# wjmaddox/online_gp

Hardware: AMD Instinct MI355X
Metric: streaming updates/sec (WISKI, 50^3 inducing grid) (higher is better)
Workload: dtype f32

## Files before the change

online_gp_amd/csrc/solve.hip:

```cpp
#include "pcg.h"

#include <hip/hip_ext.h>

#include <chrono>
#include <cstdlib>
#include <map>
#include <mutex>
#include <vector>

static struct WiskiProf {
  bool on = false;
  bool armed = false;
  std::vector<hipEvent_t> ev;
  size_t used = 0;
  unsigned long long* d_stamp = nullptr;
  size_t stamp_pairs = 0, stamp_used = 0;
  struct Span { size_t off, n; };
  std::vector<Span> spans;
} g_prof;
constexpr unsigned long long PROF_CLOCK_MASK = 0xffffffffffffull;
constexpr size_t PROF_STAMP_ARENA_PAIRS = (size_t)1 << 20;

extern "C" int wiski_prof_start(int max_launches) {
  if (max_launches < 1) return WISKI_E_BADARG;
// ... 1831 lines not shown
  return WISKI_OK;
}

template <typename real>
static int pcg_iterate(const PcgPlan<real>& plan) {
  const GridDev<real>& G = plan.G;
  const PcgArgs<real>& a = plan.a;
  const PcgLayout<real>& L = plan.L;
  const PcgScal& S = L.S;
  const hipStream_t s = plan.s;
  const int m = plan.m, k = plan.k, max_iter = a.max_iter;
  const double tol2 = plan.tol2;
  const bool spectral = plan.path.spectral;
  real *const r = plan.r, *const p = L.p, *const pt = L.pt, *const hp = L.hp, *const cpart = plan.cpart;
  const int cnch = plan.cnch, czl = plan.czl;
  wiski_pcg_async* const as = a.handle;
  int mode = a.mode, first_check = a.first_check;
  const int check_every = a.check_every < 1 ? 10 : a.check_every;
  int rc = WISKI_OK;

  std::vector<double> h_rn0(k), h_rn(k);
  double err_seen = 0;
  int dev = 0;
  if (hipGetDevice(&dev) != hipSuccess) return WISKI_E_LAUNCH;
  std::unique_lock<std::mutex> poll_lock(g_poll_mu, std::defer_lock);
  WiskiPoll* Pp = nullptr;
  if (as) {
    if (!as->poll) as->poll = new WiskiPoll();
    Pp = static_cast<WiskiPoll*>(as->poll);
  } else {
    poll_lock.lock();
    Pp = &g_polls[dev];
  }
  WiskiPoll& P = *Pp;
  if (poll_reserve(P, k) != WISKI_OK) return WISKI_E_LAUNCH;
  auto collect = [&]() {
    for (int c = 0; c < k; ++c) {
      h_rn0[c] = P.h[1 + c];
      h_rn[c] = P.h[1 + k + c];
    }
    err_seen = P.h[1 + 2 * k];
  };
  bool deferred = false;
  auto fetch = [&](int slot, long long queued_seq = 0) -> int {
    long long seq = queued_seq;
    if (!seq) {
      seq = ++P.seq;
      hipLaunchKernelGGL(k_pcg_publish, dim3(1), dim3(64), 0, s, S, slot, P.d, a.d_err, seq, tol2, P.g);
    }
    if (hipGetLastError() != hipSuccess) return WISKI_E_LAUNCH;
    if (mode == 1) {
      as->state = 1;
      as->it = slot;
      as->seq = seq;
      deferred = true;
      return WISKI_OK;
    }
    if (int prc = poll_wait(P, seq, s)) return prc;
    collect();
    return WISKI_OK;
  };
  auto converged = [&]() {
    for (int c = 0; c < k; ++c)
      if (h_rn0[c] > 0 && h_rn[c] > tol2 * h_rn0[c]) return false;
    return true;
  };

  int it = 0;
  bool done = false;
  if (mode == 2) {
    it = as->it;
    as->state = 0;
    if (int prc = poll_wait(P, as->seq, s)) return prc;
    collect();
    as->guard_ok = (long long)P.h[2 + 2 * k] == as->seq ? 1 : 0;
    done = converged();
    first_check = it;
    mode = 0;
  }
  if (first_check < 1) first_check = check_every;
  if (first_check > max_iter) first_check = max_iter;
  auto due = [&](int i) { return i == max_iter || i == first_check || (i > first_check && (i - first_check) % check_every == 0); };
  bool pending = false;
  auto flush_update = [&](bool publish = false) -> long long {
    long long seq = 0;
    if (pending) {
      if (publish) seq = ++P.seq;
      hipLaunchKernelGGL((k_pcg_update_x<real, 4>), plan.vgrid, dim3(256), 0, s, m, it - 1, tol2, (const real*)p, (const real*)pt, (const real*)hp,
                         cpart, cnch, czl, a.U, a.Z, r, S, publish ? P.d : (double*)nullptr, a.d_err, seq, P.g);
      pending = false;
    }
    return seq;
  };
  while (!done && it < max_iter) {
    if (plan.path.fused_cg) {
      constexpr bool fuse_upd = sizeof(real) == 4;
      if (!fuse_upd) flush_update();
      const bool init_now = plan.init_in_fwd && it == 0;
      rc = launch_spectral_fused_cg<real>(G, a.evec, a.evec2, a.eval, a.kscale, a.shift, r, k, L.sa, L.sb, it, pending ? 1 : 0, tol2, p, pt, cpart, cnch,
                                          czl, a.U, a.Z, S, s, init_now ? a.RHS : (const real*)nullptr, a.two_level);
      pending = false;
      if (rc) return rc;
      rc = plan.product_wide(p, pt, (real)1, S.php(it));
      if (rc) return rc;
      pending = true;
      ++it;
      if (due(it)) {
        rc = fetch(it, flush_update(true));
        if (rc) return rc;
        if (deferred) return WISKI_PENDING;
        done = converged();
      }
      continue;
    }
    if (spectral) {
      rc = launch_spectral_precond<real>(G, a.evec, a.evec2, a.eval, a.kscale, a.shift, r, k, L.sa, L.sb, L.ty, S.rho(it), s);
      if (rc) return rc;
      PCG_VEC_LAUNCH(plan, k_pcg_update_p, m, it, tol2, (const real*)(L.ty + (int64_t)k * m), (const real*)L.ty, p, pt, S);
    } else {
      rc = launch_kron<real>(G, a.tcol, r, k, a.kscale, L.tmp, L.y, r, S.rho(it), s);
      if (rc) return rc;
      PCG_VEC_LAUNCH(plan, k_pcg_update_p, m, it, tol2, (const real*)L.y, (const real*)r, p, pt, S);
    }
    rc = plan.product(p, pt, (real)1, S.php(it));
    if (rc) return rc;
    const bool pub = due(it + 1);
    const long long useq = pub ? ++P.seq : 0;
    PCG_VEC_LAUNCH(plan, k_pcg_update_x, m, it, tol2, (const real*)p, (const real*)pt, (const real*)hp, cpart, cnch, czl, a.U, a.Z, r, S,
                   pub ? P.d : (double*)nullptr, a.d_err, useq, P.g);
    ++it;
    if (due(it)) {
      rc = fetch(it, useq);
      if (rc) return rc;
      if (deferred) return WISKI_PENDING;
      done = converged();
    }
  }
  flush_update();
  if (hipGetLastError() != hipSuccess) return WISKI_E_LAUNCH;
  if (it == 0) {
    rc = fetch(0);
    if (rc) return rc;
  }
  if (a.h_iters) *a.h_iters = it;
  if (a.h_err) *a.h_err = (int32_t)err_seen;
  if (a.h_relres)
    for (int c = 0; c < k; ++c) a.h_relres[c] = h_rn0[c] > 0 ? sqrt(h_rn[c] / h_rn0[c]) : 0.0;
  return done ? WISKI_OK : WISKI_E_NOTCONV;
}
#undef PCG_VEC_LAUNCH

template <typename real>
int pcg(const wiski_grid* grid, const PcgArgs<real>& a, void* stream) {
  GridDev<real> G;
  int rc = make_grid_dev<real>(grid, &G);
  if (rc) return rc;
  const PcgPath path(G, a);
  rc = pcg_validate(G, a, path);
  if (rc) return rc;
  const PcgPlan<real> plan(G, a, path, (hipStream_t)stream);
  if (a.mode != 2) rc = pcg_start(plan);
  return rc ? rc : pcg_iterate(plan);
}
template int pcg<float>(const wiski_grid*, const PcgArgs<float>&, void*);
template int pcg<double>(const wiski_grid*, const PcgArgs<double>&, void*);

template <typename real>
static int spmv_impl(const wiski_grid* grid, const real* d_A, const real* d_V, int32_t k, const real* d_add, real beta, real* d_out, void* stream) {
  GridDev<real> G;
  int rc = make_grid_dev<real>(grid, &G);
  if (rc) return rc;
  if (!d_A || !d_V || !d_out || k < 1) return WISKI_E_BADARG;
  hipStream_t s = (hipStream_t)stream;
  if (G.m % 4 != 0) return launch_spmv<real>(G, d_A, d_V, k, d_add, beta, d_out, nullptr, s);
  const int nch = spmv_nch(G.d);
  const int64_t km = (int64_t)k * G.m;
  real* part = nullptr;
  if (hipMallocAsync((void**)&part, (size_t)nch * km * sizeof(real), s) != hipSuccess) return WISKI_E_LAUNCH;
  rc = launch_spmv4<real>(G, d_A, d_V, k, part, nullptr, (real)0, nullptr, s);
  if (rc == WISKI_OK) {
    int64_t blocks = (km + 255) / 256;
    if (blocks > 4096) blocks = 4096;
    hipLaunchKernelGGL((k_spmv_reduce<real>), dim3((unsigned)blocks), dim3(256), 0, s, km, nch, part, d_add, beta, d_out, 0);
    if (hipGetLastError() != hipSuccess) rc = WISKI_E_LAUNCH;
  }
  (void)hipFreeAsync(part, s);
  return rc;
}

template <typename real>
static int spmv_sym_impl(const wiski_grid* grid, const real* d_A, const real* d_V, int32_t k, const real* d_add, real beta, real* d_out, void* stream) {
// ... 147 lines not shown
```

online_gp_amd/csrc/spectral.hip:

```cpp
#include "wiski_common.h"

#include <atomic>

#ifdef SPEC_TIMING
__device__ long long g_spec_dbg[16];
#define SPEC_STAMP(i) do { if (threadIdx.x == 0 && blockIdx.x == 0 && blockIdx.y == 0) g_spec_dbg[i] = clock64(); } while (0)
#else
#define SPEC_STAMP(i) do {} while (0)
#endif
#ifndef SPEC_ABLATE
#ifndef SPEC_ST
#define SPEC_ST 32
#endif
#define SPEC_ABLATE 0
#endif

template <typename real>
struct V4 { real v[4]; };

template <typename real>
__device__ __forceinline__ V4<real> lds_read4(const real* p) {
  V4<real> r;
  if constexpr (sizeof(real) == 4) {
    float4 t = *reinterpret_cast<const float4*>(p);
// ... 810 lines not shown
          const unsigned long long mx = sMask[x];
          if ((mx >> y) & 1ull) {
            eidx[a][cc][r] = sPre[x] + __popcll(mx & ((1ull << y) - 1ull));
            f1v[a][cc][r] = 1.f / lam;
            f2v[a][cc][r] = 1.f;
            any_sel = true;
          }
        }
      }
    }
  for (; c < k; c += gridDim.y) {
    const int cn = c + gridDim.y;
    const bool more = cn < k;
    if (more) tX.issue(src + (int64_t)cn * m + (int64_t)i0 * g1 * g2, g1, g2);
    float dv[2][2][4];
    if constexpr (TL) {
      if (any_sel) {
#pragma unroll
        for (int a = 0; a < RT; ++a)
#pragma unroll
          for (int cc = 0; cc < 2; ++cc)
#pragma unroll
            for (int r = 0; r < 4; ++r) dv[a][cc][r] = eidx[a][cc][r] >= 0 ? dS[(int64_t)c * tl.r + eidx[a][cc][r]] : 0.f;
      }
    }
    spec_mfma_product<false, false, KS, RT>(sV1, bufA, wr, wc, lane, acc);
    store_tiles(bufB, SPEC_LDN);
    __syncthreads();
    spec_mfma_product<true, false, KS, RT>(bufB, sV2, wr, wc, lane, acc);
    spec_f32x4 c3[2][2];
    float rho_lane = 0.f;
#pragma unroll
    for (int a = 0; a < RT; ++a)
#pragma unroll
      for (int cc = 0; cc < 2; ++cc)
#pragma unroll
        for (int r = 0; r < 4; ++r) {
          float v = acc[a][cc][r];
          bool sel = false;
          if constexpr (TL) sel = any_sel && eidx[a][cc][r] >= 0;
          if (sel) v = dv[a][cc][r];
          else rho_lane += f2v[a][cc][r] * v * v;
          c3[a][cc][r] = v;
          acc[a][cc][r] = v * f1v[a][cc][r];
        }
    store_tiles(bufA, SPEC_LDN);
    if (rho != nullptr) {
      const double tot = block_reduce_sum((double)rho_lane, s_red);
      if (t == 0) unsafeAtomicAdd(rho + c, tot);
    }
    __syncthreads();
#pragma unroll
    for (int h = 0; h < 2; ++h) {
      spec_mfma_product<true, true, KS, RT>(bufA, sB2[h], wr, wc, lane, acc);
      store_tiles(bufB, SPEC_LDT);
      __syncthreads();
      if (h == 0) {
#pragma unroll
        for (int a = 0; a < RT; ++a)
#pragma unroll
          for (int cc = 0; cc < 2; ++cc)
#pragma unroll
            for (int r = 0; r < 4; ++r) acc[a][cc][r] = c3[a][cc][r] * f2v[a][cc][r];
        store_tiles(bufA, SPEC_LDN);
      } else if (more) {
        tX.commit(bufA, SPEC_LDT);
      }
      spec_mfma_product<true, false, KS, RT>(sB1[h], bufB, wr, wc, lane, acc);
      float* __restrict__ os = dst + ((int64_t)h * k + c) * m + (int64_t)i0 * g1 * g2;
#pragma unroll
      for (int a = 0; a < RT; ++a)
#pragma unroll
        for (int cc = 0; cc < 2; ++cc)
#pragma unroll
          for (int r = 0; r < 4; ++r) {
            const int x = wr * 16 * RT + a * 16 + l4 * 4 + r, y = wc * 32 + cc * 16 + l15;
            if (x < g1 && y < g2) os[x * g2 + y] = acc[a][cc][r];
          }
      __syncthreads();
    }
  }
}

template <int KS, int VW, int MODE>
__global__ __launch_bounds__(256) void k_spec_mode0_mfma(GridDev<float> G, const float* __restrict__ Va, const float* __restrict__ Vb, int split,
                                                         int transposed, const float* __restrict__ src, float* __restrict__ dst,
                                                         const float* __restrict__ rvec, int dot_c0, double* __restrict__ dots, int k, int it,
                                                         float* __restrict__ p, float* __restrict__ pt, PcgScal S, int apply, double tol2,
                                                         float* __restrict__ part, int nch, int zl, float* __restrict__ u, float* __restrict__ z) {
  __shared__ __attribute__((aligned(16))) float sF[64 * SPEC_LDT];
  __shared__ __attribute__((aligned(16))) float sIn[64 * SPEC_LDT];
  __shared__ double s_red[16];
  const int g0 = G.g[0], Sf = G.stride[0], m = G.m;
  const int cc = blockIdx.y;
  const int ntile = (Sf + 31) >> 5, per = (ntile + 7) >> 3;
  const int tile = (int)(blockIdx.x & 7) * per + (int)(blockIdx.x >> 3);
  if (tile >= ntile) return;
  const int s0 = tile * 32;
  const int t = threadIdx.x, lane = t & 63, w = t >> 6, wr = w >> 1, wc = w & 1;
  const int l15 = lane & 15, l4 = lane >> 4;
  const float* __restrict__ V0;
  int c = cc;
  float bt = 0.f;
  if (MODE == 1) {
    const int half = cc / k;
    c = cc - half * k;
    V0 = half == 0 ? Va : Vb;
    if (it > 0) {
      const double den = S.rho(it - 1)[c];
      bt = (float)(den > 0 ? S.rho(it)[c] / den : 0.0);
    }
  } else {
    V0 = cc < split ? Va : Vb;
  }
  SpecTile<VW> tV;
  tV.issue(V0, g0, g0);
  float4 tin[2];
  float al = 0.f;
  if (MODE == 2 && apply == 1) {
    const double den = S.php_sum(it - 1, cc);
    if (blockIdx.x == 0) pcg_dot_clear(S.php(it), cc, 1, S.k);
    if (pcg_active(S, it - 1, cc, tol2) && den > 0) al = (float)(S.rho(it - 1)[cc] / den);
  }
  float rn_part = 0.f, rhs_part = 0.f;
#pragma unroll
  for (int q = 0; q < 2; ++q) {
    const int b = (t >> 3) + 32 * q, q4 = (t & 7) * 4;
    const bool ok = b < g0 && s0 + q4 < Sf;
    const int64_t e = (int64_t)cc * m + (ok ? (int64_t)b * Sf + s0 + q4 : 0);
    tin[q] = *reinterpret_cast<const float4*>(src + e);
    if (!ok) tin[q] = make_float4(0.f, 0.f, 0.f, 0.f);
    if (MODE == 2 && apply == 2 && ok) {
      const float4 f4 = *reinterpret_cast<const float4*>(p + e), rv = tin[q];
      rhs_part += f4.x * f4.x + f4.y * f4.y + f4.z * f4.z + f4.w * f4.w;
      rn_part += rv.x * rv.x + rv.y * rv.y + rv.z * rv.z + rv.w * rv.w;
    }
    if (MODE == 2 && apply == 1 && ok) {
      const int64_t km = (int64_t)S.k * m;
      const float4 pv = *reinterpret_cast<const float4*>(p + e), ptv = *reinterpret_cast<const float4*>(pt + e);
      float4 uv = *reinterpret_cast<const float4*>(u + e), zv = *reinterpret_cast<const float4*>(z + e);
      float4 pp[8];
#pragma unroll
      for (int ch = 0; ch < 8; ++ch)
        if (ch < nch) pp[ch] = *reinterpret_cast<const float4*>(part + (int64_t)ch * km + e);
      if (zl) *reinterpret_cast<float4*>(part + (int64_t)(nch - 1) * km + e) = make_float4(0.f, 0.f, 0.f, 0.f);
      float4 hv = ptv;
#pragma unroll
      for (int ch = 0; ch < 8; ++ch)
        if (ch < nch) { hv.x += pp[ch].x; hv.y += pp[ch].y; hv.z += pp[ch].z; hv.w += pp[ch].w; }
      uv.x += al * pv.x; uv.y += al * pv.y; uv.z += al * pv.z; uv.w += al * pv.w;
      zv.x += al * ptv.x; zv.y += al * ptv.y; zv.z += al * ptv.z; zv.w += al * ptv.w;
      float4 rv = tin[q];
      rv.x -= al * hv.x; rv.y -= al * hv.y; rv.z -= al * hv.z; rv.w -= al * hv.w;
      rn_part += rv.x * rv.x + rv.y * rv.y + rv.z * rv.z + rv.w * rv.w;
      *reinterpret_cast<float4*>(u + e) = uv;
      *reinterpret_cast<float4*>(z + e) = zv;
      *reinterpret_cast<float4*>(const_cast<float*>(src) + e) = rv;
      tin[q] = rv;
    }
  }
  if (MODE == 2 && apply) {
    const double tot = block_reduce_sum((double)rn_part, s_red);
    if (t == 0) unsafeAtomicAdd(S.rn(it) + cc, tot);
    if (apply == 2) {
      const double tot0 = block_reduce_sum((double)rhs_part, s_red);
      if (t == 0) unsafeAtomicAdd(S.rn0() + cc, tot0);
    }
  }
  tV.commit(sF, transposed ? SPEC_LDN : SPEC_LDT);
#pragma unroll
  for (int q = 0; q < 2; ++q) *reinterpret_cast<float4*>(sIn + ((t >> 3) + 32 * q) * SPEC_LDT + (t & 7) * 4) = tin[q];
  __syncthreads();
  spec_f32x4 acc[2];
#pragma unroll
  for (int a = 0; a < 2; ++a)
#pragma unroll
    for (int r = 0; r < 4; ++r) acc[a][r] = 0.f;
  {
    const float* qb = sIn + l4 * SPEC_LDT + wc * 16 + l15;
    float af[KS][2], bf[KS];
    if (transposed) {
      const float* qa = sF + (wr * 32 + l15) * SPEC_LDN + l4;
#pragma unroll
      for (int i = 0; i < KS; ++i) { af[i][0] = qa[4 * i]; af[i][1] = qa[4 * i + 16 * SPEC_LDN]; }
    } else {
      const float* qa = sF + l4 * SPEC_LDT + wr * 32 + l15;
#pragma unroll
      for (int i = 0; i < KS; ++i) { af[i][0] = qa[4 * i * SPEC_LDT]; af[i][1] = qa[4 * i * SPEC_LDT + 16]; }
    }
#pragma unroll
    for (int i = 0; i < KS; ++i) bf[i] = qb[4 * i * SPEC_LDT];
#pragma unroll
    for (int i = 0; i < KS; ++i) {
      acc[0] = __builtin_amdgcn_mfma_f32_16x16x4f32(af[i][0], bf[i], acc[0], 0, 0, 0);
      acc[1] = __builtin_amdgcn_mfma_f32_16x16x4f32(af[i][1], bf[i], acc[1], 0, 0, 0);
    }
  }
  const int sidx = s0 + wc * 16 + l15;
  const bool dot = MODE == 0 && dots != nullptr && cc >= dot_c0;
  float dpart = 0.f;
  if (sidx < Sf) {
    float* __restrict__ tgt = MODE == 1 ? (cc < k ? pt : p) + (int64_t)c * m : dst + (int64_t)cc * m;
#pragma unroll
    for (int a = 0; a < 2; ++a)
#pragma unroll
      for (int r = 0; r < 4; ++r) {
        const int x = wr * 32 + a * 16 + l4 * 4 + r;
        if (x < g0) {
          const int64_t e = (int64_t)x * Sf + sidx;
          float o = acc[a][r];
          if (MODE == 1 && it > 0) o += bt * tgt[e];
          tgt[e] = o;
          if (dot) dpart += rvec[(int64_t)(cc - dot_c0) * m + e] * o;
        }
      }
  }
  if (dot) {
    const double tot = block_reduce_sum((double)dpart, s_red);
    if (t == 0) unsafeAtomicAdd(dots + (cc - dot_c0), tot);
  }
}

#define SPEC_DISPATCH_KS_VW(gmax, even, CALL) \
  do {                                        \
    if (even) {                               \
      if ((gmax) <= 16) CALL(4, 2);           \
      else if ((gmax) <= 32) CALL(8, 2);      \
      else if ((gmax) <= 48) CALL(12, 2);     \
      else if ((gmax) <= 52) CALL(13, 2);     \
      else CALL(16, 2);                       \
    } else {                                  \
      if ((gmax) <= 16) CALL(4, 1);           \
      else if ((gmax) <= 32) CALL(8, 1);      \
      else if ((gmax) <= 48) CALL(12, 1);     \
      else if ((gmax) <= 52) CALL(13, 1);     \
      else CALL(16, 1);                       \
    }                                         \
  } while (0)

template <typename real>
__global__ void k_spec_mode0_bwd_updp(GridDev<real> G, const real* __restrict__ X0, const real* __restrict__ Z0, const real* __restrict__ src, int k,
                                      int it, real* __restrict__ p, real* __restrict__ pt, PcgScal S);

template <typename real, bool DOT>
static int launch_mode0(const GridDev<real>& G, const real* Va, const real* Vb, int split, int transposed, const real* src, real* dst, int ncols,
                        const real* rvec, int dot_c0, double* dots, hipStream_t s) {
  const int g0 = G.g[0], Sf = G.stride[0];
  if constexpr (sizeof(real) == 4) {
    dim3 grd((unsigned)(8 * (((Sf + 31) / 32 + 7) / 8)), (unsigned)ncols);
#define M0(KS, VW)                                                                                                                          \
  hipLaunchKernelGGL((k_spec_mode0_mfma<KS, VW, 0>), grd, dim3(256), 0, s, G, Va, Vb, split, transposed, src, dst, rvec, dot_c0,            \
                     DOT ? dots : (double*)nullptr, 0, 0, (float*)nullptr, (float*)nullptr, PcgScal{nullptr, 0, nullptr}, 0, 0.0,         \
                     (float*)nullptr, 0, 0, (float*)nullptr, (float*)nullptr)
    SPEC_DISPATCH_KS_VW(g0, g0 % 2 == 0, M0);
#undef M0
  } else {
    const int P0 = (g0 + 3) & ~3;
    const size_t sh0 = (size_t)(P0 * P0 + P0 * SPEC_ST) * sizeof(real);
    hipLaunchKernelGGL((k_spec_mode0<real, DOT>), dim3((unsigned)((Sf + SPEC_ST - 1) / SPEC_ST), (unsigned)ncols), dim3(128), sh0, s, G, Va, Vb, split,
                       transposed, src, dst, rvec, dot_c0, dots);
  }
  return hipGetLastError() == hipSuccess ? WISKI_OK : WISKI_E_LAUNCH;
}

static int launch_mode0_fwd_upd(const GridDev<float>& G, const float* V0, float* r, float* dst, int k, int it, int apply, double tol2, float* p,
                                float* pt, float* part, int nch, int zl, float* u, float* z, PcgScal S, hipStream_t s) {
  const int g0 = G.g[0], Sf = G.stride[0];
  dim3 grd((unsigned)(8 * (((Sf + 31) / 32 + 7) / 8)), (unsigned)k);
#define M2(KS, VW)                                                                                                                        \
  hipLaunchKernelGGL((k_spec_mode0_mfma<KS, VW, 2>), grd, dim3(256), 0, s, G, V0, V0, 0, 0, (const float*)r, dst, (const float*)nullptr, 0, \
                     (double*)nullptr, k, it, p, pt, S, apply, tol2, part, nch, zl, u, z)
  SPEC_DISPATCH_KS_VW(g0, g0 % 2 == 0, M2);
#undef M2
  return hipGetLastError() == hipSuccess ? WISKI_OK : WISKI_E_LAUNCH;
}

template <typename real>
static int launch_mode0_bwd_updp(const GridDev<real>& G, const real* X0, const real* Z0, const real* src, int k, int it, real* p, real* pt,
                                 PcgScal S, hipStream_t s) {
  const int g0 = G.g[0], Sf = G.stride[0];
  if constexpr (sizeof(real) == 4) {
    dim3 grd((unsigned)(8 * (((Sf + 31) / 32 + 7) / 8)), (unsigned)(2 * k));
#define M1(KS, VW)                                                                                                                       \
  hipLaunchKernelGGL((k_spec_mode0_mfma<KS, VW, 1>), grd, dim3(256), 0, s, G, Z0, X0, 0, 1, src, (float*)nullptr, (const float*)nullptr, 0, \
                     (double*)nullptr, k, it, p, pt, S, 0, 0.0, (float*)nullptr, 0, 0, (float*)nullptr, (float*)nullptr)
    SPEC_DISPATCH_KS_VW(g0, g0 % 2 == 0, M1);
#undef M1
  } else {
    const int P0 = (g0 + 3) & ~3;
    const size_t sh0 = (size_t)(P0 * P0 + P0 * SPEC_ST) * sizeof(real);
    hipLaunchKernelGGL((k_spec_mode0_bwd_updp<real>), dim3((unsigned)((Sf + SPEC_ST - 1) / SPEC_ST), (unsigned)(2 * k)), dim3(128), sh0, s, G, X0, Z0,
                       src, k, it, p, pt, S);
  }
  return hipGetLastError() == hipSuccess ? WISKI_OK : WISKI_E_LAUNCH;
}

static int spec_cu_count() {
  static int n = 0;
  if (n == 0) {
    int dev = 0, v = 0;
    if (hipGetDevice(&dev) == hipSuccess && hipDeviceGetAttribute(&v, hipDeviceAttributeMultiprocessorCount, dev) == hipSuccess && v > 0) n = v;
    else n = 256;
  }
  return n;
}

constexpr size_t SPEC_SLAB_MFMA_LDS = (size_t)(4 * 64 * SPEC_LDT + 2 * 64 * SPEC_LDN) * sizeof(float);

template <typename real>
static int launch_slab(const GridDev<real>& G, const real* V1, const real* V2, const real* Z1, const real* Z2, const real* evals, real kscale,
                       real shift, const real* src, real* dst, int k, double* rho, hipStream_t s, const wiski_twolevel* two_level = nullptr) {
  const int g0 = G.g[0], g1 = G.g[1], g2 = G.g[2];
  if (two_level && (sizeof(real) != 4 || k < 1 || two_level->r < 1 || two_level->r > SPEC_TL_MAXR || two_level->nslab < 1 || two_level->nslab > g0 ||
                    !two_level->d_mask || !two_level->d_off || !two_level->d_pos || !two_level->d_N || !two_level->d_cs))
    return WISKI_E_BADARG;
  if (two_level && k == 1 && 2 * g0 > spec_cu_count()) return WISKI_E_BADARG;
  if (two_level && k > 1 && (!two_level->d_mc || two_level->mc_cols < k)) return WISKI_E_BADARG;
  if constexpr (sizeof(real) == 4) {
    const int gm = g1 > g2 ? g1 : g2;
    const bool even = g1 % 2 == 0 && g2 % 2 == 0;
    TwoLevelDev tl{};
    if (two_level) {
      static std::atomic<unsigned> tl_epoch{0};
      unsigned ep = ++tl_epoch;
      if (ep == 0) ep = ++tl_epoch;
      tl = TwoLevelDev{two_level->r, two_level->nslab, (const unsigned long long*)two_level->d_mask, two_level->d_off, two_level->d_pos,
                       two_level->d_N, (unsigned long long*)two_level->d_cs, ep};
    }
#define SLAB_MFMA2(KS, VW)                                                                                                                     \
  do {                                                                                                                                         \
    static bool lds_set = false;                                                         \
    if (!lds_set) {                                                                                                                            \
      for (const void* fp : {(const void*)k_spec_slab_mfma<KS, VW, 4, false>, (const void*)k_spec_slab_mfma<KS, VW, 8, false>,                \
                             (const void*)k_spec_slab_mfma<KS, VW, 4, true>, (const void*)k_spec_slab_mfma<KS, VW, 8, true>})                  \
        if (hipFuncSetAttribute(fp, hipFuncAttributeMaxDynamicSharedMemorySize, (int)SPEC_SLAB_MFMA_LDS) != hipSuccess)                        \
          return WISKI_E_LAUNCH;                                                                                                               \
      lds_set = true;                                                                                                                          \
    }                                                                                                                                          \
    if (two_level && slab_waves == 8)                                                                                                          \
      hipLaunchKernelGGL((k_spec_slab_mfma<KS, VW, 8, true>), dim3((unsigned)g0, 2, 1), dim3(512), SPEC_SLAB_MFMA_LDS, s, G, V1, V2, Z1,       \
                         Z2, evals, kscale, shift, src, dst, k, rho, tl);                                                                      \
    else if (two_level)                                                                                                                        \
      hipLaunchKernelGGL((k_spec_slab_mfma<KS, VW, 4, true>), dim3((unsigned)g0, 2, 1), dim3(256), SPEC_SLAB_MFMA_LDS, s, G, V1, V2, Z1,       \
                         Z2, evals, kscale, shift, src, dst, k, rho, tl);                                                                      \
    else if (slab_waves == 8)                                                                                                                  \
      hipLaunchKernelGGL((k_spec_slab_mfma<KS, VW, 8, false>), dim3((unsigned)g0, 2, (unsigned)k), dim3(512), SPEC_SLAB_MFMA_LDS, s, G, V1,    \
                         V2, Z1, Z2, evals, kscale, shift, src, dst, k, rho, tl);                                                              \
    else                                                                                                                                       \
      hipLaunchKernelGGL((k_spec_slab_mfma<KS, VW, 4, false>), dim3((unsigned)g0, 2, (unsigned)k), dim3(256), SPEC_SLAB_MFMA_LDS, s, G, V1,    \
                         V2, Z1, Z2, evals, kscale, shift, src, dst, k, rho, tl);                                                              \
  } while (0)
#define SLAB_MFMA(KS)              \
  do {                             \
    if (even) SLAB_MFMA2(KS, 2);   \
    else SLAB_MFMA2(KS, 1);        \
  } while (0)
    constexpr int slab_waves = 8;
    if (two_level ? k >= 2 : k >= 3) {
      const bool alt = Z1 != V1 || Z2 != V2;
      float* tl_c = two_level ? two_level->d_mc : nullptr;
      const float* tl_d = two_level ? two_level->d_mc + (int64_t)two_level->mc_cols * two_level->r : nullptr;
      if (two_level) {
        const size_t lb = tl_coef_mc_lds(g1, g2);
        static size_t lb_set = 0;
        if (lb > lb_set) {
          if (hipFuncSetAttribute((const void*)k_tl_coef_mc, hipFuncAttributeMaxDynamicSharedMemorySize, (int)lb) != hipSuccess) return WISKI_E_LAUNCH;
          lb_set = lb;
        }
// ... 91 lines not shown
  constexpr int NV = (64 * (ST / 4) + 127) / 128;
  V4<real> tin[NV];
#pragma unroll
  for (int itv = 0; itv < NV; ++itv) {
    const int t = threadIdx.x + itv * 128;
    const int b = t / (ST / 4), q4 = (t - b * (ST / 4)) * 4;
    V4<real> z4;
    z4.v[0] = z4.v[1] = z4.v[2] = z4.v[3] = (real)0;
    tin[itv] = (b < g0 && s0 + q4 < Sf) ? lds_read4<real>(sc + (int64_t)b * Sf + s0 + q4) : z4;
  }
  for (int e = threadIdx.x; e < P0 * P0; e += 128) sF[e] = (real)0;
  __syncthreads();
  ml.commit(sF, g0, P0);
#pragma unroll
  for (int itv = 0; itv < NV; ++itv) {
    const int t = threadIdx.x + itv * 128;
    const int b = t / (ST / 4), q4 = (t - b * (ST / 4)) * 4;
    if (b < P0) {
      real* d = sIn + b * ST + q4;
      d[0] = tin[itv].v[0]; d[1] = tin[itv].v[1]; d[2] = tin[itv].v[2]; d[3] = tin[itv].v[3];
    }
  }
  __syncthreads();
  const int nty = ST / 4, ntx = P0 / 4;
  const int t = threadIdx.x;
  if (t < ntx * nty) {
    const int tx = t / nty, ty = t - tx * nty;
    real acc[4][4];
    tile_product_t<real>(sF, P0, sIn, ST, P0, tx, ty, acc);
    const int sidx = s0 + 4 * ty;
    if (sidx < Sf) {
      real* __restrict__ tgt = (half == 0 ? pt : p) + (int64_t)c * m;
#pragma unroll
      for (int i = 0; i < 4; ++i) {
        const int x = 4 * tx + i;
        if (x < g0) {
          const int64_t e = (int64_t)x * Sf + sidx;
          real o[4] = {acc[i][0], acc[i][1], acc[i][2], acc[i][3]};
          if (it > 0) {
            const V4<real> old = lds_read4<real>(tgt + e);
#pragma unroll
            for (int q = 0; q < 4; ++q) o[q] += bt * old.v[q];
          }
          if constexpr (sizeof(real) == 4) {
            *reinterpret_cast<float4*>(tgt + e) = make_float4(o[0], o[1], o[2], o[3]);
          } else {
            *reinterpret_cast<double2*>(tgt + e) = make_double2(o[0], o[1]);
            *reinterpret_cast<double2*>(tgt + e + 2) = make_double2(o[2], o[3]);
          }
        }
      }
    }
  }
}

template <typename real>
bool spectral_fused_ok(const GridDev<real>& G) {
  if (G.d != 3) return false;
  for (int q = 0; q < 3; ++q)
    if (G.g[q] > 64) return false;
  if (G.stride[0] % 4 != 0) return false;
  return true;
}

template <typename real>
int launch_spectral_fused(const GridDev<real>& G, const real* evec, const real* evec2, const real* evals, real kscale, real shift, const real* r,
                          int k, real* w0, real* w1 , real* ty, double* rho, hipStream_t s) {
  const int g0 = G.g[0], g1 = G.g[1], g2 = G.g[2];
  if (!evec2) evec2 = evec;
  const real* V0 = evec;
  const real* V1 = evec + g0 * g0;
  const real* V2 = V1 + g1 * g1;
  const real* Z0 = evec2;
  const real* Z1 = evec2 + g0 * g0;
  const real* Z2 = Z1 + g1 * g1;
  if (int rc = launch_mode0<real, false>(G, V0, V0, 0, 0, r, w0, k, (const real*)nullptr, 0, (double*)nullptr, s)) return rc;
  if (int rc = launch_slab<real>(G, V1, V2, Z1, Z2, evals, kscale, shift, (const real*)w0, w1, k, (double*)nullptr, s)) return rc;
  return launch_mode0<real, true>(G, Z0, V0, k, 1, (const real*)w1, ty, 2 * k, r, k, rho, s);
}

template <typename real>
int launch_spectral_fused_cg(const GridDev<real>& G, const real* evec, const real* evec2, const real* evals, real kscale, real shift, real* r,
                             int k, real* w0, real* w1, int it, int apply, double tol2, real* p, real* pt, real* part, int nch, int zl, real* u,
                             real* z, PcgScal S, hipStream_t s, const real* rhs0, const wiski_twolevel* two_level) {
  const int g0 = G.g[0], g1 = G.g[1];
  if (!evec2) evec2 = evec;
  const real* V0 = evec;
  const real* V1 = evec + g0 * g0;
  const real* V2 = V1 + g1 * g1;
  const real* Z0 = evec2;
  const real* Z1 = evec2 + g0 * g0;
  const real* Z2 = Z1 + g1 * g1;
  if constexpr (sizeof(real) == 4) {
    if (rhs0 && apply) return WISKI_E_BADARG;
    if (int rc = launch_mode0_fwd_upd(G, V0, r, w0, k, it, rhs0 ? 2 : apply, tol2, rhs0 ? const_cast<float*>(rhs0) : p, pt, part, nch, zl, u, z, S, s))
      return rc;
  } else {
    if (apply || rhs0) return WISKI_E_BADARG;
    if (int rc = launch_mode0<real, false>(G, V0, V0, 0, 0, (const real*)r, w0, k, (const real*)nullptr, 0, (double*)nullptr, s)) return rc;
  }
  if (int rc = launch_slab<real>(G, V1, V2, Z1, Z2, evals, kscale, shift, (const real*)w0, w1, k, S.rho(it), s, two_level)) return rc;
  return launch_mode0_bwd_updp<real>(G, V0, Z0, (const real*)w1, k, it, p, pt, S, s);
}

template bool spectral_fused_ok<float>(const GridDev<float>&);
template int launch_spectral_fused_cg<float>(const GridDev<float>&, const float*, const float*, const float*, float, float, float*, int, float*,
                                             float*, int, int, double, float*, float*, float*, int, int, float*, float*, PcgScal, hipStream_t,
                                             const float*, const wiski_twolevel*);
template int launch_spectral_fused_cg<double>(const GridDev<double>&, const double*, const double*, const double*, double, double, double*, int,
                                              double*, double*, int, int, double, double*, double*, double*, int, int, double*, double*, PcgScal,
                                              hipStream_t, const double*, const wiski_twolevel*);
template bool spectral_fused_ok<double>(const GridDev<double>&);
template int launch_spectral_fused<float>(const GridDev<float>&, const float*, const float*, const float*, float, float, const float*, int, float*,
                                          float*, float*, double*, hipStream_t);
template int launch_spectral_fused<double>(const GridDev<double>&, const double*, const double*, const double*, double, double, const double*, int,
                                           double*, double*, double*, double*, hipStream_t);
```

online_gp_amd/csrc/wiski_common.h:

```cpp
#pragma once
#include <hip/hip_runtime.h>
#include <stdint.h>

#include "../../include/wiski.h"

#define WISKI_VERSION 1

template <typename real>
struct GridDev {
  int d;
  int g[WISKI_MAX_DIM];
  int stride[WISKI_MAX_DIM];
  real g0[WISKI_MAX_DIM];
  real h[WISKI_MAX_DIM];
  real hi[WISKI_MAX_DIM];
  int m;
  int T;
  int R;
};

template <typename real>
static inline int make_grid_dev(const wiski_grid* grid, GridDev<real>* out) {
  if (!grid || grid->d < 1 || grid->d > WISKI_MAX_DIM) return WISKI_E_BADARG;
  GridDev<real> G;
// ... 162 lines not shown
  if constexpr (sizeof(T) == 8) {
    const long long b = __builtin_bit_cast(long long, v);
    const int lo = __builtin_amdgcn_readlane((int)(b & 0xffffffffll), 63), hi = __builtin_amdgcn_readlane((int)(b >> 32), 63);
    return __builtin_bit_cast(T, ((long long)hi << 32) | (long long)(unsigned)lo);
  } else {
    return __builtin_bit_cast(T, __builtin_amdgcn_readlane(__builtin_bit_cast(int, v), 63));
  }
}

__device__ __forceinline__ double block_reduce_sum(double v, double* sm) {
  v = wave_reduce_sum<double>(v);
  int lane = threadIdx.x & 63, wid = threadIdx.x >> 6;
  if (lane == 0) sm[wid] = v;
  __syncthreads();
  double r = 0;
  if (threadIdx.x == 0) {
    int nw = (blockDim.x + 63) >> 6;
    for (int i = 0; i < nw; ++i) r += sm[i];
  }
  __syncthreads();
  return r;
}

#define WISKI_LAUNCH_CHECK()                          \
  do {                                                \
    if (hipGetLastError() != hipSuccess) return WISKI_E_LAUNCH; \
  } while (0)

#define WISKI_DISPATCH_D(d, CALL) \
  switch (d) {                    \
    case 1: { CALL(1); break; }   \
    case 2: { CALL(2); break; }   \
    case 3: { CALL(3); break; }   \
    case 4: { CALL(4); break; }   \
    default: return WISKI_E_BADARG; \
  }

constexpr int PCG_DOT_SLOTS = 16;
constexpr int PCG_DOT_STRIDE = 16;
constexpr int PCG_DOT_COL = PCG_DOT_SLOTS * PCG_DOT_STRIDE;
static inline bool wiski_shard_active(const wiski_shard* s) { return s && (s->nranks > 1 || (s->nranks == 1 && s->comm)); }

struct PcgScal {
  double* base;
  int k;
  double* ring;
  __host__ __device__ double* rn0() const { return base; }
  __host__ __device__ double* rho(int it) const { return base + (int64_t)k * (1 + 2 * it); }
  __host__ __device__ double* rn(int it) const { return base + (int64_t)k * (2 + 2 * it); }
  __host__ __device__ double* php(int it) const { return ring + (int64_t)(it & 1) * k * PCG_DOT_COL; }
  __device__ double php_sum(int it, int c) const {
    const double* q = php(it) + (int64_t)c * PCG_DOT_COL;
    double t = 0;
#pragma unroll
    for (int j = 0; j < PCG_DOT_SLOTS; ++j) t += q[j * PCG_DOT_STRIDE];
    return t;
  }
  static int64_t scalars(int k, int max_iter) { return (int64_t)k * (1 + 2 * (int64_t)(max_iter + 2)) + 1; }
  __host__ __device__ unsigned* ticket() const { return reinterpret_cast<unsigned*>(ring) - 2; }
  static int64_t doubles(int k, int max_iter) { return scalars(k, max_iter) + 2 * (int64_t)k * PCG_DOT_COL; }
};

__device__ __forceinline__ void pcg_dot_add(double* dots, int col, double v) {
  unsafeAtomicAdd(dots + (int64_t)col * PCG_DOT_COL + (blockIdx.x & (PCG_DOT_SLOTS - 1)) * PCG_DOT_STRIDE, v);
}
__device__ __forceinline__ void pcg_dot_clear(double* dots_next, int col0, int ncol, int k) {
  for (int idx = threadIdx.x; idx < ncol * PCG_DOT_COL; idx += blockDim.x) {
    const int c = col0 + idx / PCG_DOT_COL;
    if (c < k) dots_next[(int64_t)c * PCG_DOT_COL + idx % PCG_DOT_COL] = 0.0;
  }
}

__device__ __forceinline__ bool pcg_active(const PcgScal& S, int it, int c, double tol2) {
  const double rn0 = S.rn0()[c];
  return rn0 > 0 && S.rn(it)[c] > tol2 * rn0;
}

template <typename real>
bool spectral_fused_ok(const GridDev<real>& G);
template <typename real>
int launch_spectral_fused(const GridDev<real>& G, const real* evec, const real* evec2, const real* evals, real kscale, real shift, const real* r,
                          int k, real* w0, real* w1, real* ty, double* rho, hipStream_t s);

template <typename real>
int launch_spectral_fused_cg(const GridDev<real>& G, const real* evec, const real* evec2, const real* evals, real kscale, real shift, real* r,
                             int k, real* w0, real* w1, int it, int apply, double tol2, real* p, real* pt, real* part, int nch, int zl, real* u,
                             real* z, PcgScal S, hipStream_t s, const real* rhs0 = nullptr, const wiski_twolevel* two_level = nullptr);
```

Measured before the change: 25.16 million.

## Publish convergence status from fused forward mode-0 kernel instead of separate update launch

Result: slower. 24.82 million (-1.4%).

```diff
diff --git a/online_gp_amd/csrc/solve.hip b/online_gp_amd/csrc/solve.hip
--- a/online_gp_amd/csrc/solve.hip
+++ b/online_gp_amd/csrc/solve.hip
@@ -1937,6 +1937,9 @@
   if (first_check > max_iter) first_check = max_iter;
   auto due = [&](int i) { return i == max_iter || i == first_check || (i > first_check && (i - first_check) % check_every == 0); };
   bool pending = false;
+  const bool fwd_poll = plan.path.fused_cg && sizeof(real) == 4 && k == 1 && !plan.path.sharded;
+  bool fwd_done = fwd_poll && a.mode == 2;
+  SpecCgStage stage;
   auto flush_update = [&](bool publish = false) -> long long {
     long long seq = 0;
     if (pending) {
@@ -1952,16 +1955,32 @@
       constexpr bool fuse_upd = sizeof(real) == 4;
       if (!fuse_upd) flush_update();
       const bool init_now = plan.init_in_fwd && it == 0;
+      stage.part = fwd_done ? 2 : 0;
+      stage.poll = nullptr;
       rc = launch_spectral_fused_cg<real>(G, a.evec, a.evec2, a.eval, a.kscale, a.shift, r, k, L.sa, L.sb, it, pending ? 1 : 0, tol2, p, pt, cpart, cnch,
-                                          czl, a.U, a.Z, S, s, init_now ? a.RHS : (const real*)nullptr, a.two_level);
+                                          czl, a.U, a.Z, S, s, init_now ? a.RHS : (const real*)nullptr, a.two_level, stage);
       pending = false;
+      fwd_done = false;
       if (rc) return rc;
       rc = plan.product_wide(p, pt, (real)1, S.php(it));
       if (rc) return rc;
       pending = true;
       ++it;
       if (due(it)) {
-        rc = fetch(it, flush_update(true));
+        long long seq = 0;
+        if (fwd_poll) {
+          seq = ++P.seq;
+          stage.part = 1;
+          stage.poll = P.d; stage.err = a.d_err; stage.seq = seq; stage.guard = P.g;
+          rc = launch_spectral_fused_cg<real>(G, a.evec, a.evec2, a.eval, a.kscale, a.shift, r, k, L.sa, L.sb, it, 1, tol2, p, pt, cpart, cnch, czl, a.U,
+                                              a.Z, S, s, (const real*)nullptr, a.two_level, stage);
+          if (rc) return rc;
+          pending = false;
+          fwd_done = true;
+        } else {
+          seq = flush_update(true);
+        }
+        rc = fetch(it, seq);
         if (rc) return rc;
         if (deferred) return WISKI_PENDING;
         done = converged();
diff --git a/online_gp_amd/csrc/spectral.hip b/online_gp_amd/csrc/spectral.hip
--- a/online_gp_amd/csrc/spectral.hip
+++ b/online_gp_amd/csrc/spectral.hip
@@ -916,12 +916,20 @@
   }
 }
 
+struct Mode0Cg {
+  double* poll;
+  const int32_t* err;
+  long long seq;
+  long long* guard;
+};
+
 template <int KS, int VW, int MODE>
 __global__ __launch_bounds__(256) void k_spec_mode0_mfma(GridDev<float> G, const float* __restrict__ Va, const float* __restrict__ Vb, int split,
                                                          int transposed, const float* __restrict__ src, float* __restrict__ dst,
                                                          const float* __restrict__ rvec, int dot_c0, double* __restrict__ dots, int k, int it,
                                                          float* __restrict__ p, float* __restrict__ pt, PcgScal S, int apply, double tol2,
-                                                         float* __restrict__ part, int nch, int zl, float* __restrict__ u, float* __restrict__ z) {
+                                                         float* __restrict__ part, int nch, int zl, float* __restrict__ u, float* __restrict__ z,
+                                                         Mode0Cg cg) {
   __shared__ __attribute__((aligned(16))) float sF[64 * SPEC_LDT];
   __shared__ __attribute__((aligned(16))) float sIn[64 * SPEC_LDT];
   __shared__ double s_red[16];
@@ -993,9 +1001,14 @@
       tin[q] = rv;
     }
   }
+  const bool publish = MODE == 2 && cg.poll != nullptr;
+  double rn_prev = 0;
   if (MODE == 2 && apply) {
     const double tot = block_reduce_sum((double)rn_part, s_red);
-    if (t == 0) unsafeAtomicAdd(S.rn(it) + cc, tot);
+    if (t == 0) {
+      if (publish) rn_prev = atomicAdd(S.rn(it) + cc, tot);
+      else unsafeAtomicAdd(S.rn(it) + cc, tot);
+    }
     if (apply == 2) {
       const double tot0 = block_reduce_sum((double)rhs_part, s_red);
       if (t == 0) unsafeAtomicAdd(S.rn0() + cc, tot0);
@@ -1052,6 +1065,39 @@
   if (dot) {
     const double tot = block_reduce_sum((double)dpart, s_red);
     if (t == 0) unsafeAtomicAdd(dots + (cc - dot_c0), tot);
+  }
+  if (publish) {
+    __shared__ int s_last;
+    if (t == 0) {
+      unsigned one = 1u;
+      asm volatile("" : "+v"(one) : "v"(rn_prev));
+      const unsigned tk = atomicAdd(S.ticket(), one);
+      s_last = tk == (unsigned)ntile * gridDim.y - 1;
+    }
+    __syncthreads();
+    if (s_last) {
+      const int kk = S.k;
+      int ok = 1;
+      for (int c2 = t; c2 < kk; c2 += 256) {
+        const double r0 = __hip_atomic_load(S.rn0() + c2, __ATOMIC_RELAXED, __HIP_MEMORY_SCOPE_AGENT);
+        const double r1 = __hip_atomic_load(S.rn(it) + c2, __ATOMIC_RELAXED, __HIP_MEMORY_SCOPE_AGENT);
+        cg.poll[1 + c2] = r0;
+        cg.poll[1 + kk + c2] = r1;
+        if (r0 > 0 && r1 > tol2 * r0) ok = 0;
+      }
+      ok = __syncthreads_and(ok);
+      if (t == 0) {
+        const double ev = cg.err ? (double)*cg.err : 0.0;
+        const long long gv = (ok && ev == 0.0) ? cg.seq : -cg.seq;
+        cg.poll[1 + 2 * kk] = ev;
+        cg.poll[2 + 2 * kk] = (double)gv;
+        if (cg.guard) *cg.guard = gv;
+        __hip_atomic_store(S.ticket(), 0u, __ATOMIC_RELAXED, __HIP_MEMORY_SCOPE_AGENT);
+      }
+      __threadfence_system();
+      __syncthreads();
+      if (t == 0) __hip_atomic_store(reinterpret_cast<long long*>(cg.poll), cg.seq, __ATOMIC_RELEASE, __HIP_MEMORY_SCOPE_SYSTEM);
+    }
   }
 }
 
@@ -1085,7 +1131,7 @@
 #define M0(KS, VW)                                                                                                                          \
   hipLaunchKernelGGL((k_spec_mode0_mfma<KS, VW, 0>), grd, dim3(256), 0, s, G, Va, Vb, split, transposed, src, dst, rvec, dot_c0,            \
                      DOT ? dots : (double*)nullptr, 0, 0, (float*)nullptr, (float*)nullptr, PcgScal{nullptr, 0, nullptr}, 0, 0.0,         \
-                     (float*)nullptr, 0, 0, (float*)nullptr, (float*)nullptr)
+                     (float*)nullptr, 0, 0, (float*)nullptr, (float*)nullptr, Mode0Cg{})
     SPEC_DISPATCH_KS_VW(g0, g0 % 2 == 0, M0);
 #undef M0
   } else {
@@ -1098,12 +1144,13 @@
 }
 
 static int launch_mode0_fwd_upd(const GridDev<float>& G, const float* V0, float* r, float* dst, int k, int it, int apply, double tol2, float* p,
-                                float* pt, float* part, int nch, int zl, float* u, float* z, PcgScal S, hipStream_t s) {
+                                float* pt, float* part, int nch, int zl, float* u, float* z, PcgScal S, hipStream_t s, const Mode0Cg& cg) {
   const int g0 = G.g[0], Sf = G.stride[0];
   dim3 grd((unsigned)(8 * (((Sf + 31) / 32 + 7) / 8)), (unsigned)k);
+  if (cg.poll && k != 1) return WISKI_E_BADARG;
 #define M2(KS, VW)                                                                                                                        \
   hipLaunchKernelGGL((k_spec_mode0_mfma<KS, VW, 2>), grd, dim3(256), 0, s, G, V0, V0, 0, 0, (const float*)r, dst, (const float*)nullptr, 0, \
-                     (double*)nullptr, k, it, p, pt, S, apply, tol2, part, nch, zl, u, z)
+                     (double*)nullptr, k, it, p, pt, S, apply, tol2, part, nch, zl, u, z, cg)
   SPEC_DISPATCH_KS_VW(g0, g0 % 2 == 0, M2);
 #undef M2
   return hipGetLastError() == hipSuccess ? WISKI_OK : WISKI_E_LAUNCH;
@@ -1117,7 +1164,7 @@
     dim3 grd((unsigned)(8 * (((Sf + 31) / 32 + 7) / 8)), (unsigned)(2 * k));
 #define M1(KS, VW)                                                                                                                       \
   hipLaunchKernelGGL((k_spec_mode0_mfma<KS, VW, 1>), grd, dim3(256), 0, s, G, Z0, X0, 0, 1, src, (float*)nullptr, (const float*)nullptr, 0, \
-                     (double*)nullptr, k, it, p, pt, S, 0, 0.0, (float*)nullptr, 0, 0, (float*)nullptr, (float*)nullptr)
+                     (double*)nullptr, k, it, p, pt, S, 0, 0.0, (float*)nullptr, 0, 0, (float*)nullptr, (float*)nullptr, Mode0Cg{})
     SPEC_DISPATCH_KS_VW(g0, g0 % 2 == 0, M1);
 #undef M1
   } else {
@@ -1375,7 +1422,7 @@
 template <typename real>
 int launch_spectral_fused_cg(const GridDev<real>& G, const real* evec, const real* evec2, const real* evals, real kscale, real shift, real* r,
                              int k, real* w0, real* w1, int it, int apply, double tol2, real* p, real* pt, real* part, int nch, int zl, real* u,
-                             real* z, PcgScal S, hipStream_t s, const real* rhs0, const wiski_twolevel* two_level) {
+                             real* z, PcgScal S, hipStream_t s, const real* rhs0, const wiski_twolevel* two_level, const SpecCgStage& stage) {
   const int g0 = G.g[0], g1 = G.g[1];
   if (!evec2) evec2 = evec;
   const real* V0 = evec;
@@ -1384,14 +1431,20 @@
   const real* Z0 = evec2;
   const real* Z1 = evec2 + g0 * g0;
   const real* Z2 = Z1 + g1 * g1;
-  if constexpr (sizeof(real) == 4) {
-    if (rhs0 && apply) return WISKI_E_BADARG;
-    if (int rc = launch_mode0_fwd_upd(G, V0, r, w0, k, it, rhs0 ? 2 : apply, tol2, rhs0 ? const_cast<float*>(rhs0) : p, pt, part, nch, zl, u, z, S, s))
-      return rc;
-  } else {
-    if (apply || rhs0) return WISKI_E_BADARG;
-    if (int rc = launch_mode0<real, false>(G, V0, V0, 0, 0, (const real*)r, w0, k, (const real*)nullptr, 0, (double*)nullptr, s)) return rc;
-  }
+  if ((stage.part != 0 || stage.poll) && (sizeof(real) != 4 || k != 1)) return WISKI_E_BADARG;
+  if (stage.part != 2) {
+    if constexpr (sizeof(real) == 4) {
+      if (rhs0 && apply) return WISKI_E_BADARG;
+      const Mode0Cg cg{stage.poll, stage.err, stage.seq, stage.guard};
+      if (int rc = launch_mode0_fwd_upd(G, V0, r, w0, k, it, rhs0 ? 2 : apply, tol2, rhs0 ? const_cast<float*>(rhs0) : p, pt, part, nch, zl, u, z, S, s,
+                                        cg))
+        return rc;
+    } else {
+      if (apply || rhs0) return WISKI_E_BADARG;
+      if (int rc = launch_mode0<real, false>(G, V0, V0, 0, 0, (const real*)r, w0, k, (const real*)nullptr, 0, (double*)nullptr, s)) return rc;
+    }
+  }
+  if (stage.part == 1) return WISKI_OK;
   if (int rc = launch_slab<real>(G, V1, V2, Z1, Z2, evals, kscale, shift, (const real*)w0, w1, k, S.rho(it), s, two_level)) return rc;
   return launch_mode0_bwd_updp<real>(G, V0, Z0, (const real*)w1, k, it, p, pt, S, s);
 }
@@ -1399,10 +1452,10 @@
 template bool spectral_fused_ok<float>(const GridDev<float>&);
 template int launch_spectral_fused_cg<float>(const GridDev<float>&, const float*, const float*, const float*, float, float, float*, int, float*,
                                              float*, int, int, double, float*, float*, float*, int, int, float*, float*, PcgScal, hipStream_t,
-                                             const float*, const wiski_twolevel*);
+                                             const float*, const wiski_twolevel*, const SpecCgStage&);
 template int launch_spectral_fused_cg<double>(const GridDev<double>&, const double*, const double*, const double*, double, double, double*, int,
                                               double*, double*, int, int, double, double*, double*, double*, int, int, double*, double*, PcgScal,
-                                              hipStream_t, const double*, const wiski_twolevel*);
+                                              hipStream_t, const double*, const wiski_twolevel*, const SpecCgStage&);
 template bool spectral_fused_ok<double>(const GridDev<double>&);
 template int launch_spectral_fused<float>(const GridDev<float>&, const float*, const float*, const float*, float, float, const float*, int, float*,
                                           float*, float*, double*, hipStream_t);
diff --git a/online_gp_amd/csrc/wiski_common.h b/online_gp_amd/csrc/wiski_common.h
--- a/online_gp_amd/csrc/wiski_common.h
+++ b/online_gp_amd/csrc/wiski_common.h
@@ -268,7 +268,16 @@
 int launch_spectral_fused(const GridDev<real>& G, const real* evec, const real* evec2, const real* evals, real kscale, real shift, const real* r,
                           int k, real* w0, real* w1, real* ty, double* rho, hipStream_t s);
 
+struct SpecCgStage {
+  int part = 0;
+  double* poll = nullptr;
+  const int32_t* err = nullptr;
+  long long seq = 0;
+  long long* guard = nullptr;
+};
+
 template <typename real>
 int launch_spectral_fused_cg(const GridDev<real>& G, const real* evec, const real* evec2, const real* evals, real kscale, real shift, real* r,
                              int k, real* w0, real* w1, int it, int apply, double tol2, real* p, real* pt, real* part, int nch, int zl, real* u,
-                             real* z, PcgScal S, hipStream_t s, const real* rhs0 = nullptr, const wiski_twolevel* two_level = nullptr);
+                             real* z, PcgScal S, hipStream_t s, const real* rhs0 = nullptr, const wiski_twolevel* two_level = nullptr,
+                             const SpecCgStage& stage = SpecCgStage());
```
